# sharph/s-rack

Measured on AMD Instinct MI355X. Metric: voice-samples/sec @48 kHz offline render, higher is better.
Workload: dtype f32

## Files before the change

s-rack_amd/csrc/fused.hip.h:

```cpp
#pragma once
#include <hip/hip_runtime.h>
#include <type_traits>

#include "interp.hip.h"

#ifndef SRK_PRIO_AT1
#define SRK_PRIO_AT1 32
#endif
#ifndef SRK_PRIO_AT0
#define SRK_PRIO_AT0 56
#endif

#ifndef SRK_FM_UNROLL
#define SRK_FM_UNROLL 8
#endif

namespace srack {

struct CtlWork {
    const DevOp* ops;
    uint32_t* table;
    float* track;
    uint32_t T;
    uint32_t port;
// ... 195 lines not shown
                env = adsr_seg_step(sd, kd, seg, gate);
            const float o = vca_step(VCA_HAS_AUDIO | VCA_HAS_CV, negative, y, env);
            emit_put<kOut>(em, mix_tile, o, i, V);
            if (!kExact) {
                x = x_next;
                gate = gate_next;
            }
        }
        emit_flush<kOut>(em, mix_tile, t0, n, V);
    }
    if (!kExact) {
        sa.pos = pos_a;
        sl.pos = pos_l;
        sa.sync_last = sl.sync_last = false;
        adsr_seg_flush(sd, seg);
    }
    emit_stats_end(em);

    if (active) {
        auto put = [&](int rr, uint32_t v) { a.table[(size_t)rr * V + voice] = v; };
        put(oa.state_row + OSC_S_POS_LO, fixed_a ? fix_lo : f64_lo(sa.pos));
        put(oa.state_row + OSC_S_POS_HI, fixed_a ? fix_hi : f64_hi(sa.pos));
        put(oa.state_row + OSC_S_SYNC_LAST, sa.sync_last ? 1u : 0u);
        put(ol.state_row + OSC_S_POS_LO, f64_lo(sl.pos));
        put(ol.state_row + OSC_S_POS_HI, f64_hi(sl.pos));
        put(ol.state_row + OSC_S_SYNC_LAST, sl.sync_last ? 1u : 0u);
        const int s0 = ov.state_row;
        put(s0 + VCF_S_F, __float_as_uint(sv.f));
        put(s0 + VCF_S_P, __float_as_uint(sv.p));
        put(s0 + VCF_S_Q, __float_as_uint(sv.q));
        put(s0 + VCF_S_B0 + 0, __float_as_uint(sv.b0));
        put(s0 + VCF_S_B0 + 1, __float_as_uint(sv.b1));
        put(s0 + VCF_S_B0 + 2, __float_as_uint(sv.b2));
        put(s0 + VCF_S_B0 + 3, __float_as_uint(sv.b3));
        put(s0 + VCF_S_B0 + 4, __float_as_uint(sv.b4));
        put(s0 + VCF_S_FREQ, __float_as_uint(sv.freq));
        put(s0 + VCF_S_RES, __float_as_uint(sv.res));
        put(od.state_row + ADSR_S_PHASE, __float_as_uint(sd.phase));
        put(od.state_row + ADSR_S_MODE, (uint32_t)sd.mode);
        put(od.state_row + ADSR_S_R_VAL, __float_as_uint(sd.r_val));
        put(od.state_row + ADSR_S_FROM_A, __float_as_uint(sd.from_a_val));
        put(od.state_row + ADSR_S_GATE_LAST, sd.gate_last ? 1u : 0u);
    }
}

#ifdef SRK_WAVE_CENSUS
__device__ uint32_t* srk_census_rec;
SRK_DEV uint32_t* census_begin(uint32_t slot, uint32_t wave, bool ctl, int lane)
{
    uint32_t* rec = srk_census_rec;
    if (!rec || lane != 0) return nullptr;
    rec += (size_t)slot * 8;
    const uint64_t t = __builtin_amdgcn_s_memrealtime();
    rec[0] = (uint32_t)t;
    rec[1] = (uint32_t)(t >> 32);
    rec[4] = (uint32_t)__builtin_amdgcn_s_getreg((31 << 11) | 4);
    rec[5] = (uint32_t)__builtin_amdgcn_s_getreg((31 << 11) | 20);
    rec[6] = ctl ? 3u : 1u;
    rec[7] = wave;
    return rec;
}
SRK_DEV void census_end(uint32_t* rec)
{
    if (!rec) return;
    const uint64_t t = __builtin_amdgcn_s_memrealtime();
    rec[2] = (uint32_t)t;
    rec[3] = (uint32_t)(t >> 32);
}
SRK_DEV void census_end(uint32_t* rec, const dev::Pace& p)
{
    if (rec && p.word) rec[6] = 1u | 4u | (p.key << 3) | ((p.max_lead < 255u ? p.max_lead : 255u) << 16) | ((p.mine < 255u ? p.mine : 255u) << 24);
    census_end(rec);
}
#endif

template <uint32_t kOscAPort, uint32_t kVcfPort, bool kExact, int kOut>
__global__ __launch_bounds__(64) void render_voice_chain_track(KernelArgs a, ChainRoles r, CtlWork co)
{
    using namespace dev;
    __shared__ __attribute__((aligned(16))) float mix_tile[kMixTile];
    if (blockIdx.x < a.block0) {
        __builtin_amdgcn_s_setprio(3);
#ifdef SRK_WAVE_CENSUS
        uint32_t* crec = census_begin(a.n_waves, 0xffffffffu, true, threadIdx.x);
#endif
        ctl_gate_env<kExact>(co);
#ifdef SRK_WAVE_CENSUS
        census_end(crec);
#endif
        return;
    }
    const int lane = threadIdx.x;
#ifdef SRK_WAVE_CENSUS
    uint32_t* crec = census_begin(blockIdx.x - a.block0, blockIdx.x - a.block0, false, lane);
#endif
    const WaveMap wm = wave_map(a, lane);
    const uint32_t voice = wm.voice, vc = wm.vc, V = a.V;
    const bool active = wm.active;
    auto row = [&](int rr) { return a.table[(size_t)rr * V + vc]; };
    auto parv = [&](const DevOp& op, int k) { return op.par_row[k] >= 0 ? __uint_as_float(row(op.par_row[k])) : op.par_val[k]; };

    const DevOp& oa = a.ops[r.osc_a];
    const DevOp& ov = a.ops[r.vcf];
    const DevOp& oc = a.ops[r.vca];
    const int plane = a.ops[r.out].aux;
    const float* __restrict__ env_track = a.tracks + (size_t)r.track * a.t_stride;

    constexpr uint32_t fa = OSC_AA | kOscAPort | (kExact ? OSC_EXACT : 0u);
    OscRegs sa;
    OscConst ka;
    sa.pos = make_f64(row(oa.state_row + OSC_S_POS_LO), row(oa.state_row + OSC_S_POS_HI));
    sa.sync_last = row(oa.state_row + OSC_S_SYNC_LAST) != 0;
    ka.sr = oa.sample_rate;
    ka.val = 0.0;
    ka.delta = oa.delta_row >= 0 ? make_f64(row(oa.delta_row), row(oa.delta_row + 1)) : oa.delta;
    ka.inv_dt = inv_dt_f32(ka.delta);

    VcfRegs sv;
    const int s0 = ov.state_row;
    sv.f = __uint_as_float(row(s0 + VCF_S_F));
    sv.p = __uint_as_float(row(s0 + VCF_S_P));
    sv.q = __uint_as_float(row(s0 + VCF_S_Q));
    sv.b0 = __uint_as_float(row(s0 + VCF_S_B0 + 0));
    sv.b1 = __uint_as_float(row(s0 + VCF_S_B0 + 1));
    sv.b2 = __uint_as_float(row(s0 + VCF_S_B0 + 2));
    sv.b3 = __uint_as_float(row(s0 + VCF_S_B0 + 3));
    sv.b4 = __uint_as_float(row(s0 + VCF_S_B0 + 4));
    sv.freq = __uint_as_float(row(s0 + VCF_S_FREQ));
    sv.res = __uint_as_float(row(s0 + VCF_S_RES));
    if (a.T > 0) vcf_coeffs<!kExact>(sv, vcf_frequency(parv(ov, VCF_P_FREQ), 0.0f, parv(ov, VCF_P_EXP)), vcf_resonance(parv(ov, VCF_P_RES)));
    bool sv_fin = !kExact || vcf_nan_free(sv);
    const bool negative = parv(oc, VCA_P_NEG) != 0.0f;

    EmitOf<kOut> em = make_emit_of<kOut>(a, plane, lane);

    constexpr bool kFixed = !kExact && kOscAPort == OSC_OUT_SAW;
    COsc ca;
    FOsc fa_osc;
    float x = 0.0f;
    double pos_a = sa.pos;
    uint32_t fpos_lo = 0u, fpos_hi = 0u;
    if (kFixed) {
        const uint64_t dbits = oa.delta_row >= 0 ? ((uint64_t)row(oa.delta_row + 1) << 32) | row(oa.delta_row) : (uint64_t)__double_as_longlong(oa.delta);
        fosc_init(fa_osc, row(oa.state_row + OSC_S_POS_LO), row(oa.state_row + OSC_S_POS_HI), (uint32_t)dbits, (uint32_t)(dbits >> 32));
        fpos_lo = fa_osc.lo;
        fpos_hi = fa_osc.hi;
        if (a.T > 0) x = fosc_saw(fa_osc);
    } else if (!kExact) {
        cosc_init(ca, sa.pos, ka.delta);
        if (a.T > 0) x = cosc_step<kOscAPort>(ca);
    }
    typedef const __attribute__((address_space(4))) float CFloat;
    CFloat* env_s = (CFloat*)(uintptr_t)env_track;
    XSaw xo;
    const bool xs = kExact && kOscAPort == OSC_OUT_SAW && xsaw_usable(sa.pos, ka.delta) && vcf_nan_free(sv);
    if (xs) xsaw_init(xo, sa.pos, ka.delta);
    const uint32_t prio1_at = (uint32_t)(((uint64_t)a.T * SRK_PRIO_AT1) >> 6), prio0_at = (uint32_t)(((uint64_t)a.T * SRK_PRIO_AT0) >> 6);
    Pace pace = pace_join(a.pace, lane);
    __builtin_amdgcn_s_setprio(2);
    for (uint32_t t0 = 0; t0 < a.T; t0 += kMixRows) {
        const int n = (int)min((uint32_t)kMixRows, a.T - t0);
        if (!pace.word) {
            if (t0 >= prio1_at && t0 < prio1_at + kMixRows) __builtin_amdgcn_s_setprio(1);
            if (t0 >= prio0_at && t0 < prio0_at + kMixRows) __builtin_amdgcn_s_setprio(0);
        }
        if (xs) {
            xsaw_tile(xo, mix_tile + lane, kMixPitch, n);
            auto sample_x = [&](int i, float xin) {
                const float env = env_s[t0 + (uint32_t)i];
                float lp, bp, hp;
                vcf_step<false, true>(sv, xin, lp, bp, hp);
                const float y = kVcfPort == VCF_OUT_LP ? lp : (kVcfPort == VCF_OUT_BP ? bp : hp);
                const bool cv_pos = (uint32_t)(__float_as_int(env) - 1) < 0x7f800000u;
                const float o = (negative || cv_pos) ? y * env : 0.0f;
                emit_put<kOut>(em, mix_tile, o, i, V);
            };
            if (n == kMixRows) {
                uint32_t pace_seen;
                const bool pace_now = pace_step(pace, t0 / kMixRows, lane, pace_seen);
#pragma unroll
                for (int i0 = 0; i0 < kMixRows; i0 += 8) {
                    float xin[8];
#pragma unroll
                    for (int u = 0; u < 8; u++) xin[u] = mix_tile[(i0 + u) * kMixPitch + lane];
#pragma unroll
                    for (int u = 0; u < 8; u++) sample_x(i0 + u, xin[u]);
                }
                if (pace_now) pace_apply(pace, pace_seen);
            } else {
                for (int i = 0; i < n; i++) sample_x(i, mix_tile[i * kMixPitch + lane]);
            }
            emit_flush<kOut>(em, mix_tile, t0, n, V);
            continue;
        }
        auto sample = [&](int i) {
            const float env = env_s[t0 + (uint32_t)i];
            if (kExact) {
                float sine = 0.0f, square = 0.0f, saw = 0.0f;
                osc_step(fa, sa, ka, 0.0f, 0.0f, sine, square, saw);
                x = kOscAPort == OSC_OUT_SINE ? sine : (kOscAPort == OSC_OUT_SQUARE ? square : saw);
            }
            float lp, bp, hp;
            vcf_run<!kExact>(sv, sv_fin, x, lp, bp, hp);
            const float y = kVcfPort == VCF_OUT_LP ? lp : (kVcfPort == VCF_OUT_BP ? bp : hp);
            if (kFixed) {
                fpos_lo = fa_osc.lo;
                fpos_hi = fa_osc.hi;
                x = fosc_saw(fa_osc);
            } else if (!kExact) {
                pos_a = ca.pos;
                x = cosc_step<kOscAPort>(ca);
            }
            const bool cv_pos = (uint32_t)(__float_as_int(env) - 1) < 0x7f800000u;
            const float o = (negative || cv_pos) ? y * env : 0.0f;
            emit_put<kOut>(em, mix_tile, o, i, V);
        };
        if (n == kMixRows) {
            uint32_t pace_seen;
            const bool pace_now = pace_step(pace, t0 / kMixRows, lane, pace_seen);
#pragma unroll 32
            for (int i = 0; i < kMixRows; i++) sample(i);
            if (pace_now) pace_apply(pace, pace_seen);
        } else {
            for (int i = 0; i < n; i++) sample(i);
        }
        emit_flush<kOut>(em, mix_tile, t0, n, V);
    }
    if (!kExact) {
        sa.pos = pos_a;
        sa.sync_last = false;
    }
    if (xs) {
        sa.pos = xo.pos;
        sa.sync_last = false;
    }
    emit_stats_end(em);
    if (active) {
        auto put = [&](int rr, uint32_t v) { a.table[(size_t)rr * V + voice] = v; };
        put(oa.state_row + OSC_S_POS_LO, kFixed ? fpos_lo : f64_lo(sa.pos));
        put(oa.state_row + OSC_S_POS_HI, kFixed ? fpos_hi : f64_hi(sa.pos));
        put(oa.state_row + OSC_S_SYNC_LAST, sa.sync_last ? 1u : 0u);
        put(s0 + VCF_S_F, __float_as_uint(sv.f));
        put(s0 + VCF_S_P, __float_as_uint(sv.p));
        put(s0 + VCF_S_Q, __float_as_uint(sv.q));
        put(s0 + VCF_S_B0 + 0, __float_as_uint(sv.b0));
        put(s0 + VCF_S_B0 + 1, __float_as_uint(sv.b1));
        put(s0 + VCF_S_B0 + 2, __float_as_uint(sv.b2));
        put(s0 + VCF_S_B0 + 3, __float_as_uint(sv.b3));
        put(s0 + VCF_S_B0 + 4, __float_as_uint(sv.b4));
        put(s0 + VCF_S_FREQ, __float_as_uint(sv.freq));
        put(s0 + VCF_S_RES, __float_as_uint(sv.res));
    }
#ifdef SRK_WAVE_CENSUS
    census_end(crec, pace);
#endif
}

template <uint32_t kOscPort, int kOut>
__global__ __launch_bounds__(64) void render_voice_chain_seq(KernelArgs a, SeqRoles r)
{
    using namespace dev;
    __shared__ __attribute__((aligned(16))) float mix_tile[kMixTile];
    const int lane = threadIdx.x;
    const WaveMap wm = wave_map(a, lane);
    const uint32_t voice = wm.voice, vc = wm.vc, V = a.V;
    const bool active = wm.active;
    auto row = [&](int rr) { return a.table[(size_t)rr * V + vc]; };
    auto parv = [&](const DevOp& op, int k) { return op.par_row[k] >= 0 ? __uint_as_float(row(op.par_row[k])) : op.par_val[k]; };

    const DevOp& oo = a.ops[r.osc];
    const DevOp& ov = a.ops[r.vcf];
    const DevOp& oc = a.ops[r.vca];
    const int plane = a.ops[r.out].aux;
    const bool has_math = r.math >= 0, has_cut = r.trk_cutoff >= 0;
    const uint32_t mflags = has_math ? a.ops[r.math].flags : 0u;
    const float mconst = has_math ? parv(a.ops[r.math], MATH_P_CONST) : 0.0f;
    const float* __restrict__ pitch_track = a.tracks + (size_t)r.trk_pitch * a.t_stride;
    const float* __restrict__ cut_track = a.tracks + (size_t)(has_cut ? r.trk_cutoff : r.trk_env) * a.t_stride;
    const float* __restrict__ env_track = a.tracks + (size_t)r.trk_env * a.t_stride;

    constexpr uint32_t fo = OSC_HAS_CV | OSC_AA | kOscPort;
    OscConst ko;
    ko.sr = oo.sample_rate;
    ko.val = (double)parv(oo, OSC_P_VAL);
    ko.delta = 0.0;
    ko.inv_dt = 0.0f;
    COsc co;
    co.pos = make_f64(row(oo.state_row + OSC_S_POS_LO), row(oo.state_row + OSC_S_POS_HI));
    co.delta = 0.0;
    bool carried = false, have_pitch = false, have_cut = false;
    uint32_t seen_pitch = 0u, seen_cut = 0u;
    float cv_lane = 0.0f;

    VcfRegs sv;
    const int s0 = ov.state_row;
    sv.f = __uint_as_float(row(s0 + VCF_S_F));
    sv.p = __uint_as_float(row(s0 + VCF_S_P));
    sv.q = __uint_as_float(row(s0 + VCF_S_Q));
    sv.b0 = __uint_as_float(row(s0 + VCF_S_B0 + 0));
    sv.b1 = __uint_as_float(row(s0 + VCF_S_B0 + 1));
    sv.b2 = __uint_as_float(row(s0 + VCF_S_B0 + 2));
    sv.b3 = __uint_as_float(row(s0 + VCF_S_B0 + 3));
    sv.b4 = __uint_as_float(row(s0 + VCF_S_B0 + 4));
    sv.freq = __uint_as_float(row(s0 + VCF_S_FREQ));
    sv.res = __uint_as_float(row(s0 + VCF_S_RES));
    const float vfreq = parv(ov, VCF_P_FREQ), vexp = parv(ov, VCF_P_EXP), vres = vcf_resonance(parv(ov, VCF_P_RES));
    const uint32_t vport = ov.flags & (VCF_OUT_LP | VCF_OUT_BP | VCF_OUT_HP);
    if (!has_cut && a.T > 0) vcf_coeffs<true>(sv, vcf_frequency(vfreq, 0.0f, vexp), vres);
    const bool negative = parv(oc, VCA_P_NEG) != 0.0f;

    Emit em = make_emit(a, plane, lane);
    float* extra_row[4] = {nullptr, nullptr, nullptr, nullptr};
    float* extra_mp[4] = {nullptr, nullptr, nullptr, nullptr};
    __amdgpu_buffer_rsrc_t extra_rsrc[4];
    const float* extra_track[4] = {env_track, env_track, env_track, env_track};
#pragma unroll
    for (int e = 0; e < 4; e++) {
        if (e >= r.n_extra) continue;
        extra_track[e] = a.tracks + (size_t)r.extra_trk[e] * a.t_stride;
        if (a.frames) extra_row[e] = a.frames + (size_t)r.extra_plane[e] * a.plane_stride + wm.wave0;
        extra_rsrc[e] = __builtin_amdgcn_make_buffer_rsrc(extra_row[e], 0, 0x7fffffff, 0x00020000);
        if (a.mixpart) extra_mp[e] = a.mixpart + ((size_t)r.extra_plane[e] * a.n_waves + (blockIdx.x - a.block0)) * a.t_stride;
    }

    typedef const __attribute__((address_space(4))) float CFloat;
    CFloat* pitch_s = (CFloat*)(uintptr_t)pitch_track;
    CFloat* cut_s = (CFloat*)(uintptr_t)cut_track;
    CFloat* env_s = (CFloat*)(uintptr_t)env_track;
    CFloat* extra_s[4];
#pragma unroll
    for (int e = 0; e < 4; e++) extra_s[e] = (CFloat*)(uintptr_t)extra_track[e];
    const uint32_t l32 = (uint32_t)(lane & (kMixRows - 1));
    auto fetch = [&](const float* trk, uint32_t t0) { return trk[min(t0 + l32, a.T - 1)]; };
    float pitch_tile = fetch(pitch_track, 0), cut_tile = fetch(cut_track, 0);
    float extra_tile[4];
#pragma unroll
    for (int e = 0; e < 4; e++) extra_tile[e] = fetch(extra_track[e], 0);
    for (uint32_t t0 = 0; t0 < a.T; t0 += kMixRows) {
        const float pitch_next = fetch(pitch_track, t0 + kMixRows), cut_next = fetch(cut_track, t0 + kMixRows);
        float extra_next[4];
#pragma unroll
        for (int e = 0; e < 4; e++) extra_next[e] = fetch(extra_track[e], t0 + kMixRows);
        const int n = (int)min((uint32_t)kMixRows, a.T - t0);
        auto sample = [&](int i, bool steady_pitch, bool steady_cut) {
            if (!steady_pitch) {
                const uint32_t pb = __float_as_uint(pitch_s[t0 + (uint32_t)i]);
                if (!have_pitch || pb != seen_pitch) {
                    have_pitch = true;
                    seen_pitch = pb;
                    const float note = __uint_as_float(pb);
                    cv_lane = has_math ? math_step(mflags, note, 0.0f, mconst) : note;
                    const double delta = osc_delta_cold((double)cv_lane + ko.val, ko.sr);
                    carried = __builtin_amdgcn_ballot_w64(!(delta < 0.25)) == 0;
                    cosc_init(co, co.pos, delta);
                }
            }
            float x;
            if (steady_pitch || carried) {
                x = cosc_step<kOscPort>(co);
            } else {
                OscRegs g;
                g.pos = co.pos;
                g.sync_last = false;
                g.seen_cv = cv_lane;
                g.seen_delta = co.delta;
                float sine = 0.0f, square = 0.0f, saw = 0.0f;
                osc_step(fo, g, ko, cv_lane, 0.0f, sine, square, saw);
                x = kOscPort == OSC_OUT_SINE ? sine : (kOscPort == OSC_OUT_SQUARE ? square : saw);
                co.pos = g.pos;
            }
            if (has_cut && !steady_cut) {
                const float cutv = cut_s[t0 + (uint32_t)i];
                vcf_coeffs<true>(sv, vcf_frequency(vfreq, cutv, vexp), vres);
            }
            float lp, bp, hp;
            vcf_step<true>(sv, x, lp, bp, hp);
            const float y = vport == VCF_OUT_LP ? lp : (vport == VCF_OUT_BP ? bp : hp);
            const float env = env_s[t0 + (uint32_t)i];
            const bool cv_pos = (uint32_t)(__float_as_int(env) - 1) < 0x7f800000u;
            const float o = (negative || cv_pos) ? y * env : 0.0f;
// ... 1492 lines not shown
```

s-rack_amd/csrc/kernel_args.hip.h:

```cpp
#pragma once
#ifndef __HIPCC_RTC__
#include <cstdint>
#endif

#include "program.hpp"

namespace srack {

struct KernelArgs {
    const DevOp* ops;
    DevProgram prog;
    uint32_t* table;
    float* rings;
    float* frames;
    float* mixpart;
    const float* tracks;
    const uint32_t* seqtab;
    uint32_t V, T, n_waves;
    uint32_t lanes;
    uint64_t plane_stride;
    uint32_t t_stride;
    uint32_t block0;
    uint64_t n0;
    double* fv;
    const KernelArgs* ctl_slots;
    union {
        uint32_t* table_out;
        double* stats;
    };
    uint32_t* pace;
};

struct ChainRoles {
    int osc_a, osc_l, vcf, adsr, vca, out, track;
};

struct SeqRoles {
    int math, osc, vcf, vca, out;
    int trk_pitch, trk_cutoff, trk_env;
    int n_extra;
    int extra_plane[4], extra_trk[4];
};

}
```

s-rack_amd/csrc/render.hip:

```cpp
#include <hip/hip_runtime.h>

#include <algorithm>
#include <cstdio>
#include <cstdlib>
#include <cstring>
#include <memory>
#include <string>
#include <type_traits>
#include <vector>

#include "busfx.hip.h"
#include "fused.hip.h"
#include "interp.hip.h"
#include "jit.hpp"
#include "kernel_args.hip.h"
#include "modules.hip.h"
#include "freeverb_params.hpp"
#include "runtime.hpp"

namespace srack {


#define HIP_TRY(expr)                                                                                   \
    do {                                                                                                \
        hipError_t e_ = (expr);                                                                         \
        if (e_ != hipSuccess) {                                                                         \
            set_error(std::string(#expr) + ": " + hipGetErrorString(e_));                               \
            return SRACK_ERR_DEVICE;                                                                    \
        }                                                                                               \
    } while (0)

struct Knobs {
    uint32_t want_waves = 1024;
    uint32_t chunk_max = 4096;
    uint32_t chunk_first = 1024;
    bool debug_occ = false;
    int high_prio_ctl = 1;
    int special_ctl = 1;
    int fm_split = 1;
    int fm_block = 1;
    uint32_t fm_block_chunk = 65536;
    uint32_t fm_block_min = 4096;
    int mix_aside = 0;
    int pace = 1;
    int tick = 2;
};
static const Knobs& knobs()
{
    static const Knobs k = [] {
        Knobs v;
        auto num = [](const char* name, long lo, long hi, long dflt) {
            const char* e = getenv(name);
            if (!e || !*e) return dflt;
            char* end = nullptr;
            const long x = strtol(e, &end, 10);
            if (end == e) return dflt;
            return std::min(std::max(x, lo), hi);
        };
        v.want_waves = (uint32_t)num("SRACK_WANT_WAVES", 1, 1 << 20, 1024);
        v.chunk_max = (uint32_t)num("SRACK_CHUNK_MAX", 256, 65536, 4096);
        v.chunk_first = (uint32_t)num("SRACK_CHUNK_FIRST", 32, 4096, 1024);
        v.debug_occ = getenv("SRACK_DEBUG_OCC") != nullptr;
        v.high_prio_ctl = (int)num("SRACK_CTL_HIGH_PRIO", 0, 1, 1);
        v.special_ctl = (int)num("SRACK_SPECIAL_CTL", 0, 1, 1);
        v.fm_split = (int)num("SRACK_FM_SPLIT", 0, 1, 1);
        v.fm_block = (int)num("SRACK_FM_BLOCK", 0, 1, 1);
        v.fm_block_chunk = (uint32_t)num("SRACK_FM_BLOCK_CHUNK", 256, 65536, 65536);
        v.fm_block_min = (uint32_t)num("SRACK_FM_BLOCK_MIN", 1, 65536, 4096);
        v.tick = (int)num("SRACK_TICK", 0, 2, 2);
        v.mix_aside = (int)num("SRACK_MIX_ASIDE", 0, 1, 0);
        v.pace = (int)num("SRACK_PACE", 0, 1, 1);
        return v;
    }();
    return k;
}

struct DevProg {
    DevOp* d_ops = nullptr;
    uint32_t* d_table = nullptr;
    float* d_rings = nullptr;
    uint32_t* d_seqtab = nullptr;
    double* d_fv = nullptr;
    void release()
    {
        (void)hipFree(d_fv);
        d_fv = nullptr;
        (void)hipFree(d_ops);
        (void)hipFree(d_table);
        (void)hipFree(d_rings);
        (void)hipFree(d_seqtab);
        d_seqtab = nullptr;
        d_ops = nullptr;
        d_table = nullptr;
        d_rings = nullptr;
    }
};

struct TickSession {
    bool on = false;
    uint32_t L = 0;
    uint32_t Lmax = 0;
    uint32_t S = 0;
    uint32_t n = 0;
    uint32_t R = 0;
    uint64_t c = 0;
    uint64_t n0 = 0;
    hipStream_t st = nullptr;
    hipEvent_t done = nullptr;
    float* d_ring = nullptr;
    size_t ring_bytes = 0;
    std::vector<uint32_t*> d_copies;
    std::vector<size_t> words;
    uint64_t slots_base = 0;
    uint32_t slots_n = 0;
};
constexpr uint32_t kPaceSlices = 16;
constexpr uint32_t kTickBatch = 256, kTickFirstBatch = 8;

struct DeviceState {
    TickSession tick;
    hipStream_t mix_stream = nullptr;
    std::vector<hipEvent_t> ev_mix;
    hipEvent_t ev_mix_done = nullptr;
    DevProg voice;
    std::vector<DevProg> ctl;
    KernelArgs* d_stage_slots = nullptr;
    size_t stage_slots_cap = 0;
    std::vector<KernelArgs> h_stage_slots;
    float* d_mixpart = nullptr;
    size_t mixpart_bytes = 0;
    float* d_mixgroup = nullptr;
    size_t mixgroup_bytes = 0;
    float* d_tracks = nullptr;
    size_t tracks_bytes = 0;
    uint32_t* d_pace = nullptr;
    float* d_stat_frames = nullptr;
    size_t stat_frames_bytes = 0;
    uint32_t* d_bus_tab = nullptr;
    uint64_t bus_revision = 0;
    float* d_bus_part = nullptr;
    size_t bus_part_bytes = 0;
    bool last_bank_lds = false;
    uint32_t last_buses = 0;
    std::shared_ptr<const JitKernel> jit[5];
    bool jit_failed = false;
    bool bank_lds[5] = {false, false, false, false, false};
    std::string jit_note;
    std::vector<std::pair<hipEvent_t, hipEvent_t>> timings;
    std::vector<hipEvent_t> pool;
    const char* kernel_name = "";
    hipStream_t ctl_stream = nullptr;
    hipEvent_t ev_begin = nullptr;
    std::vector<hipEvent_t> ev_chunk;
    hipEvent_t ev_ready = nullptr;
    bool ready_pending = false;
};

void device_release(DeviceState* d)
{
    if (!d) return;
    d->voice.release();
    for (DevProg& c : d->ctl) c.release();
    (void)hipFree(d->d_stage_slots);
    (void)hipFree(d->d_mixpart);
    (void)hipFree(d->d_mixgroup);
    (void)hipFree(d->d_tracks);
    (void)hipFree(d->d_pace);
    (void)hipFree(d->d_stat_frames);
    (void)hipFree(d->d_bus_tab);
    (void)hipFree(d->d_bus_part);
    if (d->tick.done) (void)hipEventDestroy(d->tick.done);
    for (hipEvent_t e : d->ev_mix) (void)hipEventDestroy(e);
    if (d->ev_mix_done) (void)hipEventDestroy(d->ev_mix_done);
    if (d->mix_stream) (void)hipStreamDestroy(d->mix_stream);
    (void)hipFree(d->tick.d_ring);
    for (uint32_t* c : d->tick.d_copies) (void)hipFree(c);
    for (auto& p : d->timings) {
        (void)hipEventDestroy(p.first);
        (void)hipEventDestroy(p.second);
    }
    for (auto e : d->pool) (void)hipEventDestroy(e);
    for (auto e : d->ev_chunk) (void)hipEventDestroy(e);
    if (d->ev_begin) (void)hipEventDestroy(d->ev_begin);
    if (d->ev_ready) (void)hipEventDestroy(d->ev_ready);
    if (d->ctl_stream) (void)hipStreamDestroy(d->ctl_stream);
    delete d;
}

PatchHandle::~PatchHandle()
{
    device_busfx_drop(*this);
    device_release(dev);
    device_release(dev_old);
}

constexpr uint32_t kLaunchPolicyFlags = SRACK_RENDER_SPECIALIZE | SRACK_RENDER_NO_SPECIALIZE;

static bool program_current(const PatchHandle& h, uint32_t flags)
{
    return h.prog_valid && h.prog_graph_revision == h.graph.revision && h.prog_voices_revision == h.voices_revision && h.prog_flags == (flags & ~kLaunchPolicyFlags);
}

int peek_program(PatchHandle& h, uint32_t flags, FlatPair& scratch, const FlatPair** out)
{
    if (program_current(h, flags)) {
        *out = &h.prog;
        return SRACK_OK;
    }
    Graph g = h.graph;
    const int rc = flatten(g, h.n_voices, h.overrides, (flags & ~kLaunchPolicyFlags) | (h.keep_state ? kFlattenEvalAll : 0u), scratch);
    *out = &scratch;
    return rc;
}

static int tick_end(PatchHandle& h, hipStream_t on, bool host_wait)
{
    DeviceState* d = h.dev;
    if (!d || !d->tick.on) return SRACK_OK;
    TickSession& k = d->tick;
    if (k.done) HIP_TRY(hipStreamWaitEvent(on, k.done, 0));
    for (size_t s2 = 0; s2 < k.d_copies.size(); s2++)
        if (k.words[s2] > 0)
            HIP_TRY(hipMemcpyAsync(d->ctl[s2].d_table, k.d_copies[s2] + (size_t)(k.c % k.R) * k.words[s2], sizeof(uint32_t) * k.words[s2], hipMemcpyDeviceToDevice, on));
    k.on = false;
// ... 841 lines not shown
                    kp.block0 = n_stages;
                    kp.ctl_slots = d->d_stage_slots + (size_t)g * n_stages;
                    if ((rc = jit_launch(*special, kp, n_stages, st)) != SRACK_OK) return rc;
                }
            }
        } else if (tick && !co_ctl && tk.c + n_chunks > tk.slots_base + tk.slots_n) {
            if ((rc = tick_upload_slots(tk.c)) != SRACK_OK) return rc;
        }
        if (tick) {
        } else if (special && special_ctl) {
            if ((rc = upload_stage_slots(st)) != SRACK_OK) return rc;
            for (uint32_t j = 0; j <= max_lag && j < n_ctl_launch; j++) {
                KernelArgs kp{};
                kp.block0 = n_stages;
                kp.ctl_slots = d->d_stage_slots + (size_t)j * n_stages;
                if ((rc = jit_launch(*special, kp, n_stages, st)) != SRACK_OK) return rc;
            }
        } else if (co_ctl) {
            hipLaunchKernelGGL(render_ctl_gate_env, dim3(1), dim3(64), 0, st, ctl_work(chunks[0].first, chunks[0].second));
            HIP_TRY(hipGetLastError());
        } else if (has_ctl) {
            if (!d->ctl_stream) {
                int prio_lo = 0, prio_hi = 0;
                if (knobs().high_prio_ctl && hipDeviceGetStreamPriorityRange(&prio_lo, &prio_hi) == hipSuccess && prio_hi != prio_lo)
                    HIP_TRY(hipStreamCreateWithPriority(&d->ctl_stream, hipStreamNonBlocking, prio_hi));
                else
                    HIP_TRY(hipStreamCreateWithFlags(&d->ctl_stream, hipStreamNonBlocking));
            }
            if (!d->ev_begin) HIP_TRY(hipEventCreateWithFlags(&d->ev_begin, hipEventDisableTiming));
            while (d->ev_chunk.size() < n_chunks) {
                hipEvent_t e;
                HIP_TRY(hipEventCreateWithFlags(&e, hipEventDisableTiming));
                d->ev_chunk.push_back(e);
            }
            HIP_TRY(hipEventRecord(d->ev_begin, st));
            HIP_TRY(hipStreamWaitEvent(d->ctl_stream, d->ev_begin, 0));
            const bool staged = h.prog.ctl[0].fused == FUSED_NONE;
            if (staged) {
                const uint32_t n_launch = n_ctl_launch;
                size_t lds = 0;
                for (uint32_t s2 = 0; s2 < n_stages; s2++) lds = std::max(lds, interp_lds_bytes(h.prog.ctl[s2].hdr));
                if ((rc = upload_stage_slots(d->ctl_stream)) != SRACK_OK) return rc;
                for (uint32_t j = 0; j < n_launch; j++) {
                    const KernelArgs* slots = d->d_stage_slots + (size_t)j * n_stages;
                    if (flags & SRACK_RENDER_EXACT_OSC)
                        hipLaunchKernelGGL(render_interp_stages<true>, dim3(n_stages), dim3(64), lds, d->ctl_stream, slots);
                    else
                        hipLaunchKernelGGL(render_interp_stages<false>, dim3(n_stages), dim3(64), lds, d->ctl_stream, slots);
                    HIP_TRY(hipGetLastError());
                    if (j >= max_lag) HIP_TRY(hipEventRecord(d->ev_chunk[j - max_lag], d->ctl_stream));
                }
            } else {
                for (uint32_t k = 0; k < n_chunks; k++) {
                    launch_ctl(h.prog.ctl[0], stage_args(0, k), d->ctl_stream);
                    HIP_TRY(hipGetLastError());
                    HIP_TRY(hipEventRecord(d->ev_chunk[k], d->ctl_stream));
                }
            }
        }

        return SRACK_OK;
    }

    void pick_roles()
    {
        const bool track = pick.kernel == Kernel::VoiceChainTrack;
        if (track || pick.kernel == Kernel::VoiceChain) {
            for (int i = 0; i < (int)P.ops.size(); i++) {
                const DevOp& op = P.ops[(size_t)i];
                if (op.kind == OP_VCF) { roles.vcf = i; vcf_port = op.flags & (VCF_OUT_LP | VCF_OUT_BP | VCF_OUT_HP); }
                if (op.kind == OP_ADSR) roles.adsr = i;
                if (op.kind == OP_VCA) roles.vca = i;
                if (op.kind == OP_OUT) roles.out = i;
                if (op.kind == OP_VCA && track) roles.track = P.hdr.track_id[op.in_slot[1] - kTrackSlot];
            }
            const Graph& g = h.graph;
            roles.osc_a = P.op_of_module[(size_t)g.modules[(size_t)P.ops[(size_t)roles.vcf].module].in[0].src];
            if (!track) roles.osc_l = P.op_of_module[(size_t)g.modules[(size_t)P.ops[(size_t)roles.adsr].module].in[0].src];
            osc_port = P.ops[(size_t)roles.osc_a].flags & (OSC_OUT_SINE | OSC_OUT_SQUARE | OSC_OUT_SAW);
        } else if (pick.kernel == Kernel::SeqChain) {
            seq.math = seq.trk_cutoff = -1;
            auto track_row = [&](int slot) { return P.hdr.track_id[slot - kTrackSlot]; };
            for (int i = 0; i < (int)P.ops.size(); i++) {
                const DevOp& op = P.ops[(size_t)i];
                if (op.kind == OP_MATH) { seq.math = i; seq.trk_pitch = track_row(op.in_slot[0]); }
                if (op.kind == OP_OSC) { seq.osc = i; seq_port = op.flags & (OSC_OUT_SINE | OSC_OUT_SQUARE | OSC_OUT_SAW); }
                if (op.kind == OP_VCF) { seq.vcf = i; if (op.flags & VCF_HAS_CV) seq.trk_cutoff = track_row(op.in_slot[1]); }
                if (op.kind == OP_VCA) { seq.vca = i; seq.trk_env = track_row(op.in_slot[1]); }
                if (op.kind == OP_OUT) {
                    if (op.in_slot[0] >= kTrackSlot) {
                        seq.extra_plane[seq.n_extra] = op.aux;
                        seq.extra_trk[seq.n_extra++] = track_row(op.in_slot[0]);
                    } else {
                        seq.out = i;
                    }
                }
            }
            if (seq.math < 0) seq.trk_pitch = track_row(P.ops[(size_t)seq.osc].in_slot[0]);
        } else if (pick.kernel != Kernel::Interp) {
            roles = fm_pair_roles(P);
        }
    }

    int voices()
    {
        if (d_mix) {
            m.mixpart = d->d_mixpart;
            m.mixgroup = d->d_mixgroup;
            m.mix = d_mix;
            m.T = stride;
            m.mix_stride = T_total;
            m.n_waves = n_waves;
            m.n_channels = C;
            m.n_planes = (uint32_t)P.hdr.n_planes;
            for (int c = 0; c < 8; c++) m.channel_plane[c] = P.hdr.channel_plane[c];
        }
        mix_aside = d_mix && n_chunks > 1 && knobs().mix_aside;
        if (mix_aside) {
            if (!d->mix_stream) HIP_TRY(hipStreamCreateWithFlags(&d->mix_stream, hipStreamNonBlocking));
            if (!d->ev_mix_done) HIP_TRY(hipEventCreateWithFlags(&d->ev_mix_done, hipEventDisableTiming));
            while (d->ev_mix.size() < n_chunks) {
                hipEvent_t e = nullptr;
                HIP_TRY(hipEventCreateWithFlags(&e, hipEventDisableTiming));
                d->ev_mix.push_back(e);
            }
        }
        const bool paced = pick.paced, exact = (flags & SRACK_RENDER_EXACT_OSC) != 0;
        if (paced && !d->d_pace) HIP_TRY(hipMalloc(&d->d_pace, sizeof(uint32_t) * dev::kPaceKeys * kPaceSlices));
        for (uint32_t k = 0; k < n_chunks; k++) {
            const uint32_t t_off = chunks[k].first, len = chunks[k].second;
            KernelArgs ka{};
            if (paced) {
                if (k % kPaceSlices == 0)
                    HIP_TRY(hipMemsetAsync(d->d_pace, 0, sizeof(uint32_t) * dev::kPaceKeys * std::min(kPaceSlices, n_chunks - k), st));
                ka.pace = d->d_pace + (size_t)(k % kPaceSlices) * dev::kPaceKeys;
            }
            ka.ops = d->voice.d_ops;
            ka.prog = P.hdr;
            ka.table = d->voice.d_table;
            ka.rings = d->voice.d_rings;
            ka.seqtab = d->voice.d_seqtab;
            ka.fv = d->voice.d_fv;
            ka.frames = d_frames ? d_frames + (size_t)t_off * V : nullptr;
            ka.mixpart = d_mix ? d->d_mixpart + t_off : nullptr;
            ka.tracks = tick ? tick_tracks(tk.c + k) : has_ctl ? d->d_tracks + t_off : nullptr;
            ka.plane_stride = (uint64_t)T_total * V;
            ka.t_stride = stride;
            ka.V = V;
            ka.T = len;
            ka.n_waves = n_waves;
            ka.lanes = lanes;
            ka.n0 = h.samples_rendered + t_off;
            ka.stats = fold ? nullptr : d_stats;
            if (fold_rows) {
                ka.frames = d->d_stat_frames;
                ka.plane_stride = (uint64_t)fold_rows * V;
            }
            CtlWork co{};
            if (tick && co_ctl) {
                co = tick_work(tk.c + k + 1);
                ka.block0 = 1;
            } else if (tick) {
                ka.block0 = n_stages;
                ka.ctl_slots = d->d_stage_slots + (size_t)(max_lag + 1 + (tk.c + k - tk.slots_base)) * n_stages;
            } else if (co_ctl && k + 1 < n_chunks) {
                co = ctl_work(chunks[k + 1].first, chunks[k + 1].second);
                ka.block0 = 1;
            }
            if (has_ctl && !co_ctl && !(special && special_ctl)) HIP_TRY(hipStreamWaitEvent(st, d->ev_chunk[k], 0));
            if (!tick && special && special_ctl && k + max_lag + 1 < n_ctl_launch) {
                ka.block0 = n_stages;
                ka.ctl_slots = d->d_stage_slots + (size_t)(k + max_lag + 1) * n_stages;
            }
            hipEvent_t e0 = nullptr, e1 = nullptr;
            const bool timed = h.timing_armed;
            if (timed) {
                if ((rc = get_event(e0)) != SRACK_OK || (rc = get_event(e1)) != SRACK_OK) return rc;
                HIP_TRY(hipEventRecord(e0, st));
            }
            const int out_mode = (ka.frames ? 1 : 0) | (ka.mixpart ? 2 : 0);
            if (special) {
                if ((rc = jit_launch(*special, ka, n_waves + ka.block0, st)) != SRACK_OK) return rc;
            } else {
                switch (pick.kernel) {
                case Kernel::VoiceChainTrack:
#ifdef SRK_WAVE_CENSUS
                    if ((rc = census_arm(n_waves + 1, st)) != SRACK_OK) return rc;
#endif
                    [[fallthrough]];
                case Kernel::VoiceChain:
                    launch_fused(osc_port, vcf_port, exact, out_mode | (ka.stats ? kOutStats : 0), pick.kernel == Kernel::VoiceChainTrack, ka, roles, co, dim3(n_waves + ka.block0), st);
                    break;
                case Kernel::SeqChain: launch_seq(seq_port, out_mode, ka, seq, dim3(n_waves), st); break;
                case Kernel::FmPairX: launch_fm_pair_x(out_mode, ka, roles, dim3(n_waves), st); break;
                case Kernel::FmPairBlock:
                case Kernel::FmPairBlockX:
                    if ((rc = launch_fm_block(pick.kernel == Kernel::FmPairBlockX, out_mode, ka, roles, st)) != SRACK_OK) return rc;
                    break;
                case Kernel::FmPair:
                case Kernel::FmPairRing:
                case Kernel::FmPairSplit: launch_fm_pair(pick.kernel, exact, out_mode, ka, roles, dim3(n_waves), st); break;
                case Kernel::Interp: launch_interp(P, ka, st); break;
                }
            }
            HIP_TRY(hipGetLastError());
            if (fold) {
                hipLaunchKernelGGL(stats_fold, dim3((V + 255) / 256, (uint32_t)P.hdr.n_planes), dim3(256), 0, st, ka.frames, ka.plane_stride, V, len, d_stats);
                HIP_TRY(hipGetLastError());
            }
            if (d_bus) {
                const uint32_t n_seg = (uint32_t)h.bus_plan.seg_end.size();
                for (uint32_t r0 = 0; r0 < len; r0 += bus_slab) {
                    const uint32_t rows = std::min(bus_slab, len - r0);
                    const BusFoldArgs b = bus_args(ka.frames + (size_t)r0 * V, ka.plane_stride, t_off + r0, rows);
                    if (n_seg > 0) hipLaunchKernelGGL(bus_fold_tiles, dim3(h.bus_plan.n_tiles, (rows + kBusRows - 1) / kBusRows, (uint32_t)P.hdr.n_planes), dim3(64), 0, st, b);
                    hipLaunchKernelGGL(bus_fold_sum, dim3(h.n_buses * ((rows + 255) / 256)), dim3(256), 0, st, b);
                    HIP_TRY(hipGetLastError());
                }
            }
            if (mix_aside && k + 1 < n_chunks) {
                HIP_TRY(hipEventRecord(d->ev_mix[k], st));
                HIP_TRY(hipStreamWaitEvent(d->mix_stream, d->ev_mix[k], 0));
                MixArgs mk = m;
                mk.t_begin = t_off;
                mk.t_end = t_off + len;
                hipLaunchKernelGGL(mix_reduce_groups, dim3((len + 255) / 256, kMixSplit), dim3(256), 0, d->mix_stream, mk);
                HIP_TRY(hipGetLastError());
            }
            if (timed) {
                HIP_TRY(hipEventRecord(e1, st));
                d->timings.emplace_back(e0, e1);
                if (d->timings.size() > 4096) {
                    d->pool.push_back(d->timings.front().first);
                    d->pool.push_back(d->timings.front().second);
                    d->timings.erase(d->timings.begin());
                }
            }
        }

        return SRACK_OK;
    }

    int mix()
    {
        if (d_mix) {
            m.t_begin = mix_aside ? chunks[n_chunks - 1].first : 0u;
            m.t_end = T;
            hipLaunchKernelGGL(mix_reduce_groups, dim3((m.t_end - m.t_begin + 255) / 256, kMixSplit), dim3(256), 0, st, m);
            if (mix_aside) {
                HIP_TRY(hipEventRecord(d->ev_mix_done, d->mix_stream));
                HIP_TRY(hipStreamWaitEvent(st, d->ev_mix_done, 0));
            }
            hipLaunchKernelGGL(mix_reduce_final, dim3((T + 255) / 256), dim3(256), 0, st, m);
            HIP_TRY(hipGetLastError());
        }
        return SRACK_OK;
    }

    int finish()
    {
        h.samples_rendered += T;
        if (tick) {
            if (!tk.done) HIP_TRY(hipEventCreateWithFlags(&tk.done, hipEventDisableTiming));
            HIP_TRY(hipEventRecord(tk.done, st));
            tk.c += n_chunks;
        }
        return SRACK_OK;
    }

    int run()
    {
        bool done = false;
        if ((rc = prepare(done)) != SRACK_OK || done) return rc;
        struct TickGuard {
            PatchHandle& h;
            TickSession& t;
            bool done = false;
            ~TickGuard()
            {
                if (done || !t.on) return;
                (void)hipDeviceSynchronize();
                t.on = false;
                h.prog_valid = false;
            }
        } tick_guard{h, tk};
        if ((rc = plan()) != SRACK_OK || (rc = control()) != SRACK_OK) return rc;
        d->kernel_name = pick.name;
        pick_roles();
        if ((rc = voices()) != SRACK_OK || (rc = mix()) != SRACK_OK || (rc = finish()) != SRACK_OK) return rc;
        tick_guard.done = true;
        return SRACK_OK;
    }
};

static int render_segment(PatchHandle& h, uint32_t T_total, uint32_t t_seg, uint32_t T, float* d_frames, float* d_mix, double* d_stats, float* d_bus, uint32_t flags, hipStream_t st)
{
    if (!h.dev) {
        const int rc = upload_program(h);
        if (rc != SRACK_OK) return rc;
    }
    if (h.dev->ready_pending) {
        HIP_TRY(hipStreamWaitEvent(st, h.dev->ev_ready, 0));
        h.dev->ready_pending = false;
    }
    return Segment(h, T_total, t_seg, T, d_frames, d_mix, d_stats, d_bus, flags, st).run();
}
// ... 209 lines not shown
```

s-rack_amd/csrc/wave.hip.h:

```cpp
#pragma once
#ifndef __HIPCC_RTC__
#include <hip/hip_runtime.h>
#endif

#include "kernel_args.hip.h"
#include "modules.hip.h"

#ifndef SRK_FRAME_AUX
#define SRK_FRAME_AUX 2
#endif


namespace srack {

namespace dev {

SRK_DEV double make_f64(uint32_t lo, uint32_t hi) { return __hiloint2double((int)hi, (int)lo); }
SRK_DEV uint32_t f64_lo(double d) { return (uint32_t)__double2loint(d); }
SRK_DEV uint32_t f64_hi(double d) { return (uint32_t)__double2hiint(d); }

SRK_DEV float readlane_f32(float v, int lane) { return __int_as_float(__builtin_amdgcn_readlane(__float_as_int(v), lane)); }

SRK_DEV bool track_flat(const float* p, int lane)
{
// ... 23 lines not shown
    m.n_active = min(a.lanes, a.V - m.wave0);
    m.active = (uint32_t)lane < m.n_active;
    m.voice = m.wave0 + (uint32_t)lane;
    m.vc = m.active ? m.voice : m.wave0 + m.n_active - 1;
    return m;
}

#ifndef SRK_PACE_TILES
#define SRK_PACE_TILES 4
#endif
#ifndef SRK_PACE_LEAD
#define SRK_PACE_LEAD 1
#endif
constexpr uint32_t kPaceKeys = 8192;
constexpr uint32_t kPaceMember = 1u << 24;

struct Pace {
    uint32_t* word;
    uint32_t mine;
#ifdef SRK_WAVE_CENSUS
    uint32_t key, max_lead;
#endif
};

SRK_DEV uint32_t pace_key()
{
    const uint32_t hw = (uint32_t)__builtin_amdgcn_s_getreg((31 << 11) | 4);
    const uint32_t xcc = (uint32_t)__builtin_amdgcn_s_getreg((31 << 11) | 20);
    return ((xcc & 7u) << 10) | (((hw >> 8) & 0xffu) << 2) | ((hw >> 4) & 3u);
}

SRK_DEV Pace pace_join(uint32_t* slice, int lane)
{
    Pace p{};
    if (!slice) return p;
    const uint32_t key = pace_key();
    p.word = slice + key;
    if (lane == 0) atomicAdd(p.word, kPaceMember);
#ifdef SRK_WAVE_CENSUS
    p.key = key;
#endif
    return p;
}

SRK_DEV bool pace_step(Pace& p, uint32_t tile, int lane, uint32_t& seen)
{
    seen = 0u;
    if (!p.word || tile == 0u || tile % SRK_PACE_TILES != 0u) return false;
    p.mine++;
    if (lane == 0) seen = atomicAdd(p.word, 1u);
    return true;
}

SRK_DEV void pace_apply(Pace& p, uint32_t seen)
{
    const uint32_t got = (uint32_t)__builtin_amdgcn_readfirstlane((int)seen);
    const int n = (int)(got >> 24);
    const int lead = n * (int)p.mine - (int)((got & (kPaceMember - 1u)) + 1u);
    const int band = SRK_PACE_LEAD * (n > 2 ? n - 1 : 1);
    if (lead >= band)
        __builtin_amdgcn_s_setprio(0);
    else if (lead <= -band)
        __builtin_amdgcn_s_setprio(2);
    else
        __builtin_amdgcn_s_setprio(1);
#ifdef SRK_WAVE_CENSUS
    const uint32_t al = (uint32_t)(lead < 0 ? -lead : lead);
    p.max_lead = al > p.max_lead ? al : p.max_lead;
#endif
}

}

constexpr int kMixRows = 32;
static_assert(kMixRows == dev::kTileRows, "the tile-wise module forms (modules.hip.h) assume the mix tile's length");
constexpr int kMixPitch = 68;
constexpr int kMixTile = kMixRows * kMixPitch;

constexpr int kStatCount = 6;
enum { kStatSum = 0, kStatSumSq = 1, kStatPeakPos = 2, kStatPeakNeg = 3, kStatNonfinite = 4, kStatClipped = 5 };

struct VoiceStats {
    double sum, sum_sq;
    float peak_pos, peak_neg;
    uint32_t nonfinite, clipped;
};

SRK_DEV void stats_add(VoiceStats& s, float x)
{
    const bool fin = __builtin_isfinite(x);
    const float xs = fin ? x : -0.0f;
    const double xd = (double)xs;
    s.sum += xd;
    s.sum_sq = __builtin_fma(xd, xd, s.sum_sq);
    s.peak_pos = xs > s.peak_pos ? xs : s.peak_pos;
    s.peak_neg = -xs > s.peak_neg ? -xs : s.peak_neg;
    s.nonfinite += fin ? 0u : 1u;
    s.clipped += fabsf(xs) > 1.0f ? 1u : 0u;
}

SRK_DEV void stats_load(VoiceStats& s, const double* p, size_t V)
{
    s.sum = p[(size_t)kStatSum * V];
    s.sum_sq = p[(size_t)kStatSumSq * V];
    s.peak_pos = (float)p[(size_t)kStatPeakPos * V];
    s.peak_neg = (float)p[(size_t)kStatPeakNeg * V];
    s.nonfinite = s.clipped = 0u;
}
SRK_DEV void stats_store(const VoiceStats& s, double* p, size_t V)
{
    p[kStatSum * V] = s.sum;
    p[kStatSumSq * V] = s.sum_sq;
    p[kStatPeakPos * V] = (double)s.peak_pos;
    p[kStatPeakNeg * V] = (double)s.peak_neg;
    p[kStatNonfinite * V] += (double)s.nonfinite;
    p[kStatClipped * V] += (double)s.clipped;
}

struct Emit {
    float* frame_row;
    __amdgpu_buffer_rsrc_t rsrc;
    uint32_t soff;
    float* mp;
    bool has_frames, has_mix, full_wave;
    int lane, lane_c;
    uint32_t n_active;
};

constexpr int kOutStats = 8;
struct EmitStats : Emit {
    double* stats;
    uint32_t stats_stride;
    VoiceStats st;
};
template <bool kStats>
struct EmitSel { typedef Emit type; };
template <>
struct EmitSel<true> { typedef EmitStats type; };
template <int kOut>
using EmitOf = typename EmitSel<(kOut & kOutStats) != 0>::type;

template <int kOut, class E>
SRK_DEV void emit_put(E& e, float* mix_tile, float o, int i, uint32_t V)
{
    const bool frames = (kOut & ~kOutStats) == 0 ? e.has_frames : (kOut & 1) != 0;
    const bool mix = (kOut & ~kOutStats) == 0 ? e.has_mix : (kOut & 2) != 0;
    if (frames) {
        __builtin_amdgcn_raw_buffer_store_b32(__float_as_uint(o), e.rsrc, e.lane_c * 4, (int)e.soff, SRK_FRAME_AUX);
        e.soff += V * 4u;
    }
    if (mix) mix_tile[i * kMixPitch + e.lane] = o;
    if constexpr ((kOut & kOutStats) != 0) stats_add(e.st, o);
}

SRK_DEV void emit_rebase(Emit& e)
{
    e.rsrc = __builtin_amdgcn_make_buffer_rsrc(e.frame_row, 0, 0x7fffffff, 0x00020000);
    e.soff = 0u;
}

template <int kOut, bool kBarrier = true>
SRK_DEV void emit_flush(Emit& e, float* mix_tile, uint32_t t0, int n, uint32_t V)
{
    const bool frames = (kOut & ~kOutStats) == 0 ? e.has_frames : (kOut & 1) != 0;
    if (frames) {
        e.frame_row += (size_t)n * V;
        emit_rebase(e);
    }
    const bool mix = (kOut & ~kOutStats) == 0 ? e.has_mix : (kOut & 2) != 0;
    if (!mix) return;
    if (!e.full_wave && (uint32_t)e.lane >= e.n_active)
        for (int r = 0; r < kMixRows; r++) mix_tile[r * kMixPitch + e.lane] = 0.0f;
    if (kBarrier) __syncthreads();
    typedef float f4 __attribute__((ext_vector_type(4)));
    const f4* p = (const f4*)(mix_tile + (e.lane & 31) * kMixPitch + (e.lane >> 5) * 32);
    f4 acc = p[0];
#pragma unroll
    for (int q = 1; q < 8; q++) acc += p[q];
    float sum = (acc.x + acc.y) + (acc.z + acc.w);
    sum += __shfl_xor(sum, 32);
    if (e.lane < n) e.mp[t0 + e.lane] = sum;
    if (kBarrier) __syncthreads();
}

template <int kOut>
SRK_DEV void emit_put_rows(Emit& e, float* rows, float o, int r, uint32_t V)
{
    const bool frames = kOut == 0 ? e.has_frames : (kOut & 1) != 0;
    const bool mix = kOut == 0 ? e.has_mix : (kOut & 2) != 0;
    if (frames) {
        __builtin_amdgcn_raw_buffer_store_b32(__float_as_uint(o), e.rsrc, e.lane_c * 4, (int)e.soff, SRK_FRAME_AUX);
        e.soff += V * 4u;
    }
    if (mix) rows[r * kMixPitch + e.lane] = o;
}
template <int kRows>
SRK_DEV void emit_rows_flush(const Emit& e, float* tile, float* mp_lane, uint32_t t_first, int n_valid)
{
    static_assert(kRows == 16 || kRows == 8 || kRows == 4, "rows per plane");
    if (!e.full_wave && (uint32_t)e.lane >= e.n_active)
        for (int r = 0; r < kMixRows; r++) tile[r * kMixPitch + e.lane] = 0.0f;
    __syncthreads();
    typedef float f4 __attribute__((ext_vector_type(4)));
    const f4* p = (const f4*)(tile + (e.lane & 31) * kMixPitch + (e.lane >> 5) * 32);
    f4 acc = p[0];
#pragma unroll
    for (int q = 1; q < 8; q++) acc += p[q];
    float sum = (acc.x + acc.y) + (acc.z + acc.w);
    sum += __shfl_xor(sum, 32);
    const int r = e.lane & (kRows - 1);
    if (e.lane < 32 && r < n_valid && mp_lane) mp_lane[t_first + (uint32_t)r] = sum;
    __syncthreads();
}
template <int kOut>
SRK_DEV void emit_rows_end(Emit& e, int n, uint32_t V)
{
    const bool frames = kOut == 0 ? e.has_frames : (kOut & 1) != 0;
    if (frames) {
        e.frame_row += (size_t)n * V;
        emit_rebase(e);
    }
}

SRK_DEV void emit_track_put(Emit& e, float v, uint32_t V, bool frames)
{
    if (frames) {
        __builtin_amdgcn_raw_buffer_store_b32(__float_as_uint(v), e.rsrc, e.lane_c * 4, (int)e.soff, SRK_FRAME_AUX);
        e.soff += V * 4u;
    }
}
SRK_DEV void emit_track_flush(Emit& e, const float* track_t0, uint32_t t0, int n, uint32_t V, bool frames, bool mix)
{
    if (frames) {
        e.frame_row += (size_t)n * V;
        emit_rebase(e);
    }
    if (mix && e.lane < n) e.mp[t0 + e.lane] = (float)e.n_active * track_t0[e.lane];
}

SRK_DEV void emit_stats_begin(EmitStats& e, const KernelArgs& a, int plane)
{
    const uint32_t V = a.V;
    e.stats = a.stats + (size_t)plane * kStatCount * V + (size_t)(dev::wave_index(a) * a.lanes + (uint32_t)e.lane_c);
    e.stats_stride = V;
    stats_load(e.st, e.stats, V);
}
SRK_DEV void emit_stats_end(const Emit&) {}
SRK_DEV void emit_stats_end(const EmitStats& e)
{
    if ((uint32_t)e.lane >= e.n_active) return;
    stats_store(e.st, e.stats, e.stats_stride);
}

SRK_DEV Emit make_emit(const KernelArgs& a, int plane, int lane)
{
    using dev::WaveMap;
    using dev::wave_map;
    Emit e;
    const WaveMap wm = wave_map(a, lane);
    const uint32_t wave0 = wm.wave0;
    e.n_active = wm.n_active;
    e.full_wave = e.n_active == 64u;
    e.lane = lane;
    e.lane_c = min(lane, (int)e.n_active - 1);
    e.frame_row = a.frames ? a.frames + (size_t)plane * a.plane_stride + wave0 : nullptr;
    e.mp = a.mixpart ? a.mixpart + ((size_t)plane * a.n_waves + (blockIdx.x - a.block0)) * a.t_stride : nullptr;
    e.has_frames = e.frame_row != nullptr;
    e.has_mix = e.mp != nullptr;
    emit_rebase(e);
    return e;
}

template <int kOut>
SRK_DEV EmitOf<kOut> make_emit_of(const KernelArgs& a, int plane, int lane)
{
    if constexpr ((kOut & kOutStats) != 0) {
        EmitStats e;
        static_cast<Emit&>(e) = make_emit(a, plane, lane);
        emit_stats_begin(e, a, plane);
        return e;
    } else {
        return make_emit(a, plane, lane);
    }
}

}
```

Measured before the change: 1249 billion.

## Skip per-sample envelope gating on all-positive tiles and batch envelope scalar loads

Restructures the fused osc→VCF→VCA tile loop. A wave-wide ballot over the next tile's envelope bits decides whether every sample is positive, and if so a gate-free path drops the per-sample compare and select. Envelope values are now fetched eight at a time as uniform scalar vector loads, prefetched ahead of use, with an asm pin that keeps the store offset in an SGPR. The change adds a runtime knob, extra code paths that may raise register pressure, and a per-tile lookahead load and ballot.

```diff
diff --git a/s-rack_amd/csrc/fused.hip.h b/s-rack_amd/csrc/fused.hip.h
--- a/s-rack_amd/csrc/fused.hip.h
+++ b/s-rack_amd/csrc/fused.hip.h
@@ -371,80 +371,115 @@
     }
     typedef const __attribute__((address_space(4))) float CFloat;
     CFloat* env_s = (CFloat*)(uintptr_t)env_track;
+    const uint32_t* env_bits = (const uint32_t*)env_track;
+    const uint32_t l32 = (uint32_t)lane & (uint32_t)(kMixRows - 1);
+    const uint32_t gate_force = a.tile_plain != 0u ? 0u : 0x80000000u;
+    auto all_pos = [&](uint32_t bits) { return __builtin_amdgcn_ballot_w64(!(((bits | gate_force) - 1u) < 0x7f800000u)) == 0; };
+    bool plain = a.T >= (uint32_t)kMixRows && all_pos(env_bits[l32]);
     XSaw xo;
     const bool xs = kExact && kOscAPort == OSC_OUT_SAW && xsaw_usable(sa.pos, ka.delta) && vcf_nan_free(sv);
     if (xs) xsaw_init(xo, sa.pos, ka.delta);
     const uint32_t prio1_at = (uint32_t)(((uint64_t)a.T * SRK_PRIO_AT1) >> 6), prio0_at = (uint32_t)(((uint64_t)a.T * SRK_PRIO_AT0) >> 6);
     Pace pace = pace_join(a.pace, lane);
     __builtin_amdgcn_s_setprio(2);
-    for (uint32_t t0 = 0; t0 < a.T; t0 += kMixRows) {
-        const int n = (int)min((uint32_t)kMixRows, a.T - t0);
+    auto sample_x = [&](int i, float xin, float env, bool gated, bool pinned) __attribute__((always_inline)) {
+        float lp, bp, hp;
+        vcf_step<false, true>(sv, xin, lp, bp, hp);
+        const float y = kVcfPort == VCF_OUT_LP ? lp : (kVcfPort == VCF_OUT_BP ? bp : hp);
+        const bool cv_pos = (uint32_t)(__float_as_int(env) - 1) < 0x7f800000u;
+        const float o = (!gated || negative || cv_pos) ? y * env : 0.0f;
+        emit_put<kOut>(em, mix_tile, o, i, V);
+        if (pinned) emit_row_pin<kOut>(em);
+    };
+    auto sample = [&](int i, float env, bool gated, bool pinned) __attribute__((always_inline)) {
+        if (kExact) {
+            float sine = 0.0f, square = 0.0f, saw = 0.0f;
+            osc_step(fa, sa, ka, 0.0f, 0.0f, sine, square, saw);
+            x = kOscAPort == OSC_OUT_SINE ? sine : (kOscAPort == OSC_OUT_SQUARE ? square : saw);
+        }
+        float lp, bp, hp;
+        vcf_run<!kExact>(sv, sv_fin, x, lp, bp, hp);
+        const float y = kVcfPort == VCF_OUT_LP ? lp : (kVcfPort == VCF_OUT_BP ? bp : hp);
+        if (kFixed) {
+            fpos_lo = fa_osc.lo;
+            fpos_hi = fa_osc.hi;
+            x = fosc_saw(fa_osc);
+        } else if (!kExact) {
+            pos_a = ca.pos;
+            x = cosc_step<kOscAPort>(ca);
+        }
+        const bool cv_pos = (uint32_t)(__float_as_int(env) - 1) < 0x7f800000u;
+        const float o = (!gated || negative || cv_pos) ? y * env : 0.0f;
+        emit_put<kOut>(em, mix_tile, o, i, V);
+        if (pinned) emit_row_pin<kOut>(em);
+    };
+    auto full_tile = [&](uint32_t t0, auto kX, bool gated) __attribute__((always_inline)) {
         if (!pace.word) {
             if (t0 >= prio1_at && t0 < prio1_at + kMixRows) __builtin_amdgcn_s_setprio(1);
             if (t0 >= prio0_at && t0 < prio0_at + kMixRows) __builtin_amdgcn_s_setprio(0);
         }
-        if (xs) {
-            xsaw_tile(xo, mix_tile + lane, kMixPitch, n);
-            auto sample_x = [&](int i, float xin) {
-                const float env = env_s[t0 + (uint32_t)i];
-                float lp, bp, hp;
-                vcf_step<false, true>(sv, xin, lp, bp, hp);
-                const float y = kVcfPort == VCF_OUT_LP ? lp : (kVcfPort == VCF_OUT_BP ? bp : hp);
-                const bool cv_pos = (uint32_t)(__float_as_int(env) - 1) < 0x7f800000u;
-                const float o = (negative || cv_pos) ? y * env : 0.0f;
-                emit_put<kOut>(em, mix_tile, o, i, V);
-            };
-            if (n == kMixRows) {
-                uint32_t pace_seen;
-                const bool pace_now = pace_step(pace, t0 / kMixRows, lane, pace_seen);
-#pragma unroll
-                for (int i0 = 0; i0 < kMixRows; i0 += 8) {
-                    float xin[8];
-#pragma unroll
-                    for (int u = 0; u < 8; u++) xin[u] = mix_tile[(i0 + u) * kMixPitch + lane];
-#pragma unroll
-                    for (int u = 0; u < 8; u++) sample_x(i0 + u, xin[u]);
+        if (decltype(kX)::value) xsaw_tile(xo, mix_tile + lane, kMixPitch, kMixRows);
+        const uint32_t gate_next = env_bits[min(t0 + (uint32_t)kMixRows + l32, a.T - 1u)];
+        uint32_t pace_seen;
+        const bool pace_now = pace_step(pace, t0 / kMixRows, lane, pace_seen);
+        float8u e[kMixRows / 8];
+        float xin[8];
+        e[0] = uniform_load8(env_s + t0);
+#pragma unroll 32
+        for (int i = 0; i < kMixRows; i++) {
+            if ((i & 7) == 2 && i + 8 < kMixRows) e[(i >> 3) + 1] = uniform_load8(env_s + t0 + (uint32_t)((i & ~7) + 8));
+            if (decltype(kX)::value) {
+                if ((i & 7) == 0) {
+#pragma unroll
+                    for (int u = 0; u < 8; u++) xin[u] = mix_tile[(i + u) * kMixPitch + lane];
                 }
-                if (pace_now) pace_apply(pace, pace_seen);
+                sample_x(i, xin[i & 7], e[i >> 3][i & 7], gated, true);
             } else {
-                for (int i = 0; i < n; i++) sample_x(i, mix_tile[i * kMixPitch + lane]);
+                sample(i, e[i >> 3][i & 7], gated, true);
+            }
+        }
+        const uint32_t seen = (uint32_t)__builtin_amdgcn_readfirstlane((int)pace_seen);
+        if (pace_now) pace_apply(pace, seen);
+        plain = all_pos(gate_next);
+        emit_flush<kOut>(em, mix_tile, t0, kMixRows, V);
+    };
+    auto tiles = [&](auto kX) __attribute__((always_inline)) {
+        const uint32_t t_full = a.T & ~(uint32_t)(kMixRows - 1);
+        uint32_t t0 = 0;
+        constexpr bool kTwo = !kExact || decltype(kX)::value;
+        while (t0 < t_full) {
+            if (kTwo && plain) {
+                do {
+                    full_tile(t0, kX, false);
+                    t0 += kMixRows;
+                } while (t0 < t_full && plain);
+            } else {
+                do {
+                    full_tile(t0, kX, true);
+                    t0 += kMixRows;
+                } while (t0 < t_full && !(kTwo && plain));
+            }
+            __builtin_amdgcn_s_waitcnt(0x0f70);
+        }
+        if (t0 < a.T) {
+            const int n = (int)(a.T - t0);
+            if (!pace.word) {
+                if (t0 >= prio1_at && t0 < prio1_at + kMixRows) __builtin_amdgcn_s_setprio(1);
+                if (t0 >= prio0_at && t0 < prio0_at + kMixRows) __builtin_amdgcn_s_setprio(0);
+            }
+            if (decltype(kX)::value) {
+                xsaw_tile(xo, mix_tile + lane, kMixPitch, n);
+                for (int i = 0; i < n; i++) sample_x(i, mix_tile[i * kMixPitch + lane], env_s[t0 + (uint32_t)i], true, false);
+            } else {
+                for (int i = 0; i < n; i++) sample(i, env_s[t0 + (uint32_t)i], true, false);
             }
             emit_flush<kOut>(em, mix_tile, t0, n, V);
-            continue;
-        }
-        auto sample = [&](int i) {
-            const float env = env_s[t0 + (uint32_t)i];
-            if (kExact) {
-                float sine = 0.0f, square = 0.0f, saw = 0.0f;
-                osc_step(fa, sa, ka, 0.0f, 0.0f, sine, square, saw);
-                x = kOscAPort == OSC_OUT_SINE ? sine : (kOscAPort == OSC_OUT_SQUARE ? square : saw);
-            }
-            float lp, bp, hp;
-            vcf_run<!kExact>(sv, sv_fin, x, lp, bp, hp);
-            const float y = kVcfPort == VCF_OUT_LP ? lp : (kVcfPort == VCF_OUT_BP ? bp : hp);
-            if (kFixed) {
-                fpos_lo = fa_osc.lo;
-                fpos_hi = fa_osc.hi;
-                x = fosc_saw(fa_osc);
-            } else if (!kExact) {
-                pos_a = ca.pos;
-                x = cosc_step<kOscAPort>(ca);
-            }
-            const bool cv_pos = (uint32_t)(__float_as_int(env) - 1) < 0x7f800000u;
-            const float o = (negative || cv_pos) ? y * env : 0.0f;
-            emit_put<kOut>(em, mix_tile, o, i, V);
-        };
-        if (n == kMixRows) {
-            uint32_t pace_seen;
-            const bool pace_now = pace_step(pace, t0 / kMixRows, lane, pace_seen);
-#pragma unroll 32
-            for (int i = 0; i < kMixRows; i++) sample(i);
-            if (pace_now) pace_apply(pace, pace_seen);
-        } else {
-            for (int i = 0; i < n; i++) sample(i);
-        }
-        emit_flush<kOut>(em, mix_tile, t0, n, V);
-    }
+        }
+    };
+    if (xs)
+        tiles(std::true_type{});
+    else
+        tiles(std::false_type{});
     if (!kExact) {
         sa.pos = pos_a;
         sa.sync_last = false;
diff --git a/s-rack_amd/csrc/kernel_args.hip.h b/s-rack_amd/csrc/kernel_args.hip.h
--- a/s-rack_amd/csrc/kernel_args.hip.h
+++ b/s-rack_amd/csrc/kernel_args.hip.h
@@ -29,6 +29,7 @@
         double* stats;
     };
     uint32_t* pace;
+    uint32_t tile_plain;
 };
 
 struct ChainRoles {
diff --git a/s-rack_amd/csrc/render.hip b/s-rack_amd/csrc/render.hip
--- a/s-rack_amd/csrc/render.hip
+++ b/s-rack_amd/csrc/render.hip
@@ -43,6 +43,7 @@
     uint32_t fm_block_min = 4096;
     int mix_aside = 0;
     int pace = 1;
+    int tile_plain = 1;
     int tick = 2;
 };
 static const Knobs& knobs()
@@ -70,6 +71,7 @@
         v.tick = (int)num("SRACK_TICK", 0, 2, 2);
         v.mix_aside = (int)num("SRACK_MIX_ASIDE", 0, 1, 0);
         v.pace = (int)num("SRACK_PACE", 0, 1, 1);
+        v.tile_plain = (int)num("SRACK_TILE_PLAIN", 0, 1, 1);
         return v;
     }();
     return k;
@@ -1217,6 +1219,7 @@
             ka.lanes = lanes;
             ka.n0 = h.samples_rendered + t_off;
             ka.stats = fold ? nullptr : d_stats;
+            ka.tile_plain = (uint32_t)knobs().tile_plain;
             if (fold_rows) {
                 ka.frames = d->d_stat_frames;
                 ka.plane_stride = (uint64_t)fold_rows * V;
diff --git a/s-rack_amd/csrc/wave.hip.h b/s-rack_amd/csrc/wave.hip.h
--- a/s-rack_amd/csrc/wave.hip.h
+++ b/s-rack_amd/csrc/wave.hip.h
@@ -199,6 +199,16 @@
     if (mix) mix_tile[i * kMixPitch + e.lane] = o;
     if constexpr ((kOut & kOutStats) != 0) stats_add(e.st, o);
 }
+
+template <int kOut>
+SRK_DEV void emit_row_pin(Emit& e)
+{
+    if constexpr ((kOut & ~kOutStats) != 2) asm("" : "+s"(e.soff));
+}
+
+typedef float float8u __attribute__((ext_vector_type(8)));
+typedef float8u float8u_dw __attribute__((aligned(4)));
+SRK_DEV float8u uniform_load8(const __attribute__((address_space(4))) float* p) { return *(const __attribute__((address_space(4))) float8u_dw*)p; }
 
 SRK_DEV void emit_rebase(Emit& e)
 {
```

Result: faster. 1280 billion, median of 6 (+2.5%).
